# netsys-lab/scion-xdp-br

Measured on AMD Instinct MI355X. Metric: Mpkt/s device-resident hop-field AES-CMAC verify, 64 B SCION packets, higher is better.
Workload: dtype u8; 1 GPU; config 2: 1048576 x 64 B records per GPU per step, single AS key; records_per_gpu=1048576, record_bytes=64, keysel=zero, resident_batches_per_gpu=8, resident_bytes_per_gpu=536870912, parallelism=batch-sharded x1, no collective

## Files before the change

scion-xdp-br_amd/csrc/hfv_aes_dev.h:

```cpp
#pragma once
#include <hip/hip_runtime.h>

#include "hfv_internal.h"

namespace hfv {
#define T0V(i) kTables.t0[i]
#define T0V8(i) T0V(i), T0V(i + 1), T0V(i + 2), T0V(i + 3), T0V(i + 4), T0V(i + 5), T0V(i + 6), T0V(i + 7)
#define T0V64(i) T0V8(i), T0V8(i + 8), T0V8(i + 16), T0V8(i + 24), T0V8(i + 32), T0V8(i + 40), T0V8(i + 48), T0V8(i + 56)
static __constant__ uint32_t c_t0[256] = {T0V64(0), T0V64(64), T0V64(128), T0V64(192)};
#undef T0V64
#undef T0V8
#undef T0V


static __shared__ uint32_t s_tab64[16384];
static __shared__ uint32_t s_tab128[32768];
constexpr uint32_t kTab3Copies = 8;
constexpr uint32_t kTab3Log = kTab3Copies == 32 ? 5 : kTab3Copies == 16 ? 4 : kTab3Copies == 8 ? 3 : kTab3Copies == 4 ? 2 : 99;
static_assert(kTab3Log < 8, "kTab3Copies must be 4, 8, 16 or 32");
static __shared__ uint32_t s_tab32[256 * 2 * kTab3Copies];
static __shared__ uint4 s_keys[kDevKeyRows * HFV_MAX_KEYS];
static __shared__ uint32_t s_valid[8];
static __shared__ uint32_t s_next_tile;

constexpr uint32_t sel_byte(int k) { return 0x0c020400u | (uint32_t(k) << 8); }
constexpr uint32_t SEL_B0 = sel_byte(0), SEL_B1 = sel_byte(1), SEL_B2 = sel_byte(2), SEL_B3 = sel_byte(3);

__device__ __forceinline__ uint32_t rot16(uint32_t x) { return __builtin_amdgcn_alignbit(x, x, 16); }

struct Lane;
template <int TAB, int K>
__device__ __forceinline__ uint32_t tlu(uint32_t w, uint32_t base, const Lane &l);

template <int TAB>
__device__ __forceinline__ void fill_ttab()
{
    if constexpr (TAB == 3) {
#pragma unroll 4
        for (int e = threadIdx.x; e < (int)(256 * 2 * kTab3Copies); e += blockDim.x) {
            uint32_t t = c_t0[(e >> kTab3Log) & 255];
            s_tab32[e] = (e >> (kTab3Log + 8)) ? __builtin_amdgcn_alignbit(t, t, 24) : t;
        }
        return;
    }
    constexpr int kDwords = TAB == 4 ? 32768 : 16384;
    uint32_t *dst = TAB == 4 ? s_tab128 : s_tab64;
#pragma unroll 4
    for (int e = threadIdx.x; e < kDwords; e += blockDim.x) {
        uint32_t t = c_t0[(e >> 6) & 255];
        int rot = 8 * (((e >> 5) & 1) | ((e >> 13) & 2));
        dst[e] = rot ? __builtin_amdgcn_alignbit(t, t, 32 - rot) : t;
    }
}

template <int TAB, class P>
__device__ __forceinline__ void fill_ttab_karg(P t0, uint32_t wave, uint32_t nw)
{
    constexpr uint32_t kChunks = (TAB == 4 ? 131072 : 65536) / 1024;
    constexpr int kMax = (int)((kChunks + 14) / 15);
    const uint32_t lane = threadIdx.x & 63;
    char *lds = TAB == 4 ? reinterpret_cast<char *>(s_tab128) : reinterpret_cast<char *>(s_tab64);
    uint32_t v[kMax];
#pragma unroll
    for (int k = 0; k < kMax; ++k) {
        const uint32_t c = wave + k * nw;
        const uint32_t e = (c << 3) + (lane >> 3);
        v[k] = c < kChunks ? t0[(e >> 1) & 255u] : 0u;
    }
#pragma unroll
    for (int k = 0; k < kMax; ++k) {
        const uint32_t c = wave + k * nw;
        if (c < kChunks) {
            const uint32_t e = (c << 3) + (lane >> 3);
            const uint32_t t = (e & 1u) | (((e >> 9) & 1u) << 1);
            const uint32_t x = t ? __builtin_amdgcn_alignbit(v[k], v[k], 32 - 8 * t) : v[k];
            *reinterpret_cast<uint4 *>(lds + c * 1024 + lane * 16) = make_uint4(x, x, x, x);
        }
    }
}

__device__ __forceinline__ void fill_keys(const DevKeyTable *tab, uint32_t nthr = 0)
{
    const uint32_t n = nthr ? nthr : blockDim.x;
    const uint4 *src = reinterpret_cast<const uint4 *>(tab->rows);
    for (uint32_t e = threadIdx.x; e < kDevKeyRows * HFV_MAX_KEYS; e += n) s_keys[e] = src[e];
    if (threadIdx.x < 8) s_valid[threadIdx.x] = tab->valid[threadIdx.x];
}

struct Lane {
    uint32_t b0, b1, b2, b3;
    uint32_t s0, s1, s2, s3;
    uint32_t f01, f23;
};

template <int TAB, int K>
__device__ __forceinline__ uint32_t tlu(uint32_t w, uint32_t base, const Lane &l)
{
    static_assert(K >= 0 && K < 4, "state byte");
    if constexpr (TAB == 3) {
        const uint32_t a3 = (__builtin_amdgcn_ubfe(w, 8 * K, 8) << (kTab3Log + 2)) | base;
        return *reinterpret_cast<const uint32_t *>(reinterpret_cast<const char *>(s_tab32) + a3);
    }
    const uint32_t a = __builtin_amdgcn_perm(w, base, K == 0 ? l.s0 : K == 1 ? l.s1 : K == 2 ? l.s2 : l.s3);
    const char *t = TAB == 4 ? reinterpret_cast<const char *>(s_tab128) : reinterpret_cast<const char *>(s_tab64);
    return *reinterpret_cast<const uint32_t *>(t + a);
}

__device__ __forceinline__ uint32_t vconst(uint32_t c)
{
    uint32_t r;
    asm("v_mov_b32 %0, %1" : "=v"(r) : "i"(c));
    return r;
}

__device__ __forceinline__ uint32_t xor3(uint32_t a, uint32_t b, uint32_t c)
{
    return __builtin_amdgcn_bitop3_b32(a, b, c, 0x96);
}

template <int TAB, bool PIN = false>
__device__ __forceinline__ void round_full(uint32_t s[4], const uint4 &rk, const Lane &l)
{
    const uint32_t r[4] = {rk.x, rk.y, rk.z, rk.w};
    uint32_t n[4];
#pragma unroll
    for (int c = 0; c < 4; ++c) {
        uint32_t a = tlu<TAB, 0>(s[c], l.b0, l);
        uint32_t b = tlu<TAB, 1>(s[(c + 1) & 3], l.b1, l);
        if constexpr (TAB == 4) {
            uint32_t x = tlu<TAB, 2>(s[(c + 2) & 3], l.b2, l);
            uint32_t d = tlu<TAB, 3>(s[(c + 3) & 3], l.b3, l);
            n[c] = xor3(xor3(a, b, x), d, r[c]);
        } else {
            uint32_t x = tlu<TAB, 2>(s[(c + 2) & 3], l.b0, l);
            uint32_t d = tlu<TAB, 3>(s[(c + 3) & 3], l.b1, l);
            n[c] = xor3(a, b, rot16(xor3(x, d, r[c])));
        }
    }
#pragma unroll
    for (int c = 0; c < 4; ++c) s[c] = n[c];
    if constexpr (TAB == 4 && PIN) {
        __builtin_amdgcn_sched_group_barrier(0x002, 16, 0);
        __builtin_amdgcn_sched_group_barrier(0x100, 16, 0);
        __builtin_amdgcn_sched_group_barrier(0x002, 8, 0);
    }
}

template <int TAB>
__device__ __forceinline__ void round1_macinput(uint32_t s[4], const uint4 &rk1p, const Lane &l)
{
    uint32_t n0, n1, n2, n3;
    if constexpr (TAB == 4) {
        n0 = xor3(tlu<TAB, 1>(s[1], l.b1, l), tlu<TAB, 2>(s[2], l.b2, l), rk1p.x);
        n1 = xor3(xor3(tlu<TAB, 0>(s[1], l.b0, l), tlu<TAB, 1>(s[2], l.b1, l), tlu<TAB, 3>(s[0], l.b3, l)), rk1p.y, 0u);
        n2 = xor3(xor3(tlu<TAB, 1>(s[3], l.b1, l), tlu<TAB, 2>(s[0], l.b2, l), tlu<TAB, 3>(s[1], l.b3, l)), rk1p.z, 0u);
        n3 = xor3(xor3(tlu<TAB, 0>(s[3], l.b0, l), tlu<TAB, 2>(s[1], l.b2, l), tlu<TAB, 3>(s[2], l.b3, l)), rk1p.w, 0u);
    } else {
        n0 = xor3(tlu<TAB, 1>(s[1], l.b1, l), rot16(tlu<TAB, 2>(s[2], l.b0, l)), rk1p.x);
        n1 = xor3(tlu<TAB, 0>(s[1], l.b0, l), tlu<TAB, 1>(s[2], l.b1, l), rk1p.y) ^ rot16(tlu<TAB, 3>(s[0], l.b1, l));
        n2 = xor3(tlu<TAB, 1>(s[3], l.b1, l), rot16(tlu<TAB, 2>(s[0], l.b0, l) ^ tlu<TAB, 3>(s[1], l.b1, l)), rk1p.z);
        n3 = xor3(tlu<TAB, 0>(s[3], l.b0, l), rot16(tlu<TAB, 2>(s[1], l.b0, l) ^ tlu<TAB, 3>(s[2], l.b1, l)), rk1p.w);
    }
// ... 167 lines not shown
```

scion-xdp-br_amd/csrc/hfv_api.cpp:

```cpp
#include <stdarg.h>
#include <stdio.h>
#include <stdlib.h>

#include "hfv_ctx.h"

namespace hfv {

static thread_local char g_err[256];

int fail(int code, const char *fmt, ...)
{
    va_list ap;
    va_start(ap, fmt);
    vsnprintf(g_err, sizeof g_err, fmt, ap);
    va_end(ap);
    return code;
}

}

#ifdef HFV_TEST_HOOKS
static unsigned g_br_grid = 0;
extern "C" int hfv_debug_br_grid(unsigned blocks)
{
// ... 204 lines not shown
    return hfv_key_add(ctx, index, &k);
}

int hfv_key_remove(hfv_ctx *ctx, uint32_t index)
{
    if (!ctx) return fail(-EINVAL, "ctx is NULL");
    if (index >= HFV_MAX_KEYS) return fail(-EINVAL, "key index %u >= %d", index, HFV_MAX_KEYS);
    if (!((ctx->valid[index >> 5] >> (index & 31)) & 1u)) return fail(-ENOENT, "key slot %u is empty", index);
    if (ctx->keymap) {
        int rc = hfv_keymap_erase(ctx->keymap_path, index);
        if (rc) return rc;
    }
    ctx->valid[index >> 5] &= ~(1u << (index & 31));
    memset(&ctx->shadow[index], 0, sizeof(hop_key));
    ctx->dirty = true;
    return 0;
}

int hfv_ctx_attach_keymap(hfv_ctx *ctx, const char *path)
{
    if (!ctx || !path) return fail(-EINVAL, "null argument");
    if (strlen(path) >= sizeof ctx->keymap_path) return fail(-ENAMETOOLONG, "path too long");
    const void *m = nullptr;
    int rc = keymap_open_ro(path, &m);
    if (rc == -ENOENT) {
        rc = keymap_create(path, HFV_KEYMAP_SLOTS);
        if (!rc) rc = keymap_open_ro(path, &m);
    }
    if (rc) return fail(rc, "cannot attach key map %s", path);
    keymap_close(ctx->keymap);
    ctx->keymap = m;
    strcpy(ctx->keymap_path, path);
    ctx->keymap_seq = keymap_snapshot(m, ctx->shadow, ctx->valid);
    ctx->dirty = true;
    return 0;
}

int hfv_key_get(hfv_ctx *ctx, uint32_t index, struct hop_key *out)
{
    if (!ctx || !out) return fail(-EINVAL, "null argument");
    if (index >= HFV_MAX_KEYS) return fail(-EINVAL, "key index %u >= %d", index, HFV_MAX_KEYS);
    if (!((ctx->valid[index >> 5] >> (index & 31)) & 1u)) return fail(-ENOENT, "key slot %u is empty", index);
    *out = ctx->shadow[index];
    return 0;
}

int hfv_key_add_batch(hfv_ctx *ctx, uint32_t first, const struct aes_key *keys, size_t n)
{
    if (!ctx || (!keys && n)) return fail(-EINVAL, "null argument");
    if ((size_t)first + n > HFV_MAX_KEYS) return fail(-EINVAL, "slots %u..%zu exceed %d", first, first + n, HFV_MAX_KEYS);
    if (n == 0) return 0;
    DeviceGuard g(ctx->device);
    SVC_QUIESCE(ctx);
    uint8_t *d_raw = nullptr;
    hop_key *d_hk = nullptr;
    HIP_TRY(hipMalloc((void **)&d_raw, 16 * n));
    if (hipMalloc((void **)&d_hk, sizeof(hop_key) * n) != hipSuccess) {
        (void)hipFree(d_raw);
        return fail(-ENOMEM, "hipMalloc");
    }
    int rc = 0;
    if (hipMemcpyAsync(d_raw, keys, 16 * n, hipMemcpyHostToDevice, ctx->stream) != hipSuccess) rc = -EIO;
    if (!rc && launch_expand_keys(d_raw, n, d_hk, nullptr, 0, ctx->stream) != 0) rc = -EIO;
    hop_key *tmp = (hop_key *)malloc(sizeof(hop_key) * n);
    if (!tmp) rc = -ENOMEM;
    if (!rc && hipMemcpyAsync(tmp, d_hk, sizeof(hop_key) * n, hipMemcpyDeviceToHost, ctx->stream) != hipSuccess) rc = -EIO;
    if (!rc && hipStreamSynchronize(ctx->stream) != hipSuccess) rc = -EIO;
    if (rc) rc = fail(rc, "device key expansion failed");
    for (size_t i = 0; !rc && i < n; ++i) rc = hfv_key_set_hop_key(ctx, first + (uint32_t)i, &tmp[i]);
    free(tmp);
    (void)hipFree(d_raw);
    (void)hipFree(d_hk);
    return rc;
}


static int verify_records(hfv_ctx *ctx, const void *recs, size_t stride, size_t n, uint64_t *pass_bits, void *stream,
                          hipEvent_t ev0, hipEvent_t ev1)
{
    int rc = check_records(ctx, recs, stride, pass_bits);
    if (rc) return rc;
    DeviceGuard g(ctx->device);
    SVC_QUIESCE(ctx);
    return with_tables(ctx, (hipStream_t)stream, "verify_records launch", [&](DevState *ds) {
        return launch_verify_records(batch_geom(ctx), &ds->keys, &ctx->host_img->keys, ctx->keysel, (const uint8_t *)recs,
                                     stride, n, ctx->inf_off, ctx->hf_off, pass_bits, stream, ev0, ev1);
    });
}

int hfv_verify_records(hfv_ctx *ctx, const void *recs, size_t stride, size_t n, uint64_t *pass_bits, void *stream)
{
    if (!ctx) return fail(-EINVAL, "ctx is NULL");
    if (n == 0) return 0;
    return verify_records(ctx, recs, stride, n, pass_bits, stream, nullptr, nullptr);
}

int hfv_verify_records_timed(hfv_ctx *ctx, const void *recs, size_t stride, size_t n, uint64_t *pass_bits,
                             void *stream, float *kernel_ms)
{
    if (!ctx || !kernel_ms) return fail(-EINVAL, "null argument");
    *kernel_ms = 0.0f;
    if (n == 0) return 0;
    return timed(ctx, kernel_ms, [&](hipEvent_t ev0, hipEvent_t ev1) {
        return verify_records(ctx, recs, stride, n, pass_bits, stream, ev0, ev1);
    });
}

static int batches_check(const hfv_ctx *ctx, const struct hfv_batch *b, size_t count)
{
    if (!b && count) return fail(-EINVAL, "null batch list");
    for (size_t i = 0; i < count; ++i) {
        if (b[i].n == 0) continue;
        int rc = check_records(ctx, b[i].recs, b[i].stride, b[i].pass_bits);
        if (rc) return fail_batch(rc, i);
        if (b[i].stride > (1u << 24)) return fail(-EINVAL, "batch %zu: stride %zu > 16 MiB", i, b[i].stride);
        if (b[i].n > ((size_t)1 << 36)) return fail(-EINVAL, "batch %zu: %zu records (at most 2^36)", i, b[i].n);
    }
    return 0;
}

static int batches_launch(hfv_ctx *ctx, const struct hfv_batch *b, size_t count, hipStream_t st, hipEvent_t ev0,
                          hipEvent_t ev1)
{
    size_t last = count;
    while (last > 0 && b[last - 1].n == 0) --last;
    if (ev0) HIP_TRY(hipMemsetAsync(ctx->bat_clk + 4 + kBatchStampBlocks, 0, kBatchStampBlocks * sizeof(uint64_t), st));
    return with_tables(ctx, st, "verify_batches launch", [&](DevState *ds) {
        if (last == 0) return (int)hipSuccess;
        BatchArgs a;
        memset(&a, 0, sizeof a);
        a.tab = &ds->keys;
        a.inf_off = ctx->inf_off;
        a.hf_off = ctx->hf_off;
        a.clk = ctx->bat_clk;
        a.pro = key_prologue(&ctx->host_img->keys);
        for (size_t i = 0;;) {
            a.nb = 0;
            uint64_t tiles = 0;
            for (; i < last && a.nb < kBatchMax; ++i) {
                if (b[i].n == 0) continue;
                const uint64_t t = (b[i].n + 63) / 64;
                if (a.nb && tiles + t > (1ull << 31)) break;
                a.d[a.nb] = {(uint64_t)(uintptr_t)b[i].recs, (uint64_t)(uintptr_t)b[i].pass_bits, (uint64_t)b[i].n,
                             (uint64_t)b[i].stride};
                a.cum[a.nb] = (uint32_t)tiles;
                tiles += t;
                ++a.nb;
            }
            a.cum[a.nb] = (uint32_t)tiles;
            a.total = (uint32_t)tiles;
            const bool fin = i >= last;
            int e = launch_verify_batches(batch_geom(ctx), ctx->keysel, a, st, ev0, fin ? ev1 : nullptr);
            if (e != hipSuccess || fin) return e;
            note_reader(ctx, st);
            ev0 = nullptr;
        }
    });
}

int hfv_verify_batches(hfv_ctx *ctx, const struct hfv_batch *batches, size_t count, void *stream)
{
    if (!ctx) return fail(-EINVAL, "ctx is NULL");
    int rc = batches_check(ctx, batches, count);
    if (rc) return rc;
    DeviceGuard g(ctx->device);
    SVC_QUIESCE(ctx);
    return batches_launch(ctx, batches, count, (hipStream_t)stream, nullptr, nullptr);
}

int hfv_verify_batches_timed(hfv_ctx *ctx, const struct hfv_batch *batches, size_t count, void *stream,
                             float *kernel_ms)
{
    if (!ctx || !kernel_ms) return fail(-EINVAL, "null argument");
    *kernel_ms = 0.0f;
    int rc = batches_check(ctx, batches, count);
    if (rc) return rc;
    size_t nonempty = 0;
    for (size_t i = 0; i < count; ++i) nonempty += batches[i].n != 0;
    if (!nonempty) return 0;
    return timed(ctx, kernel_ms, [&](hipEvent_t ev0, hipEvent_t ev1) {
        SVC_QUIESCE(ctx);
        return batches_launch(ctx, batches, count, (hipStream_t)stream, ev0, ev1);
    });
}


static int frames_check(const hfv_ctx *ctx, const uint8_t *frames, size_t slot, const uint16_t *len, size_t n,
                        const void *recs, size_t stride, const uint8_t *status)
{
    if (!frames || !len || !status) return fail(-EINVAL, "null buffer");
    if ((slot & 7) || slot < 64) return fail(-EINVAL, "slot %zu: must be a multiple of 8, at least 64", slot);
    if (slot > (1u << 24)) return fail(-EINVAL, "slot %zu > 16 MiB", slot);
    int rc = check_records(ctx, recs, stride, recs);
    if (rc) return rc;
    if (stride > (1u << 24)) return fail(-EINVAL, "stride %zu > 16 MiB", stride);
    if (n > ((size_t)1 << 36)) return fail(-EINVAL, "%zu frames (at most 2^36)", n);
    return 0;
}

int hfv_ctx_set_internal_ifindices(hfv_ctx *ctx, const uint32_t *ifindex, size_t n)
{
    if (!ctx) return fail(-EINVAL, "ctx is NULL");
    if (n > kRxSetMax) return fail(-EINVAL, "%zu internal ifindices (at most %u)", n, kRxSetMax);
    if (!ifindex && n) return fail(-EINVAL, "null ifindex list");
    ctx->rx_set.n = (uint32_t)n;
    for (size_t i = 0; i < kRxSetMax; ++i) ctx->rx_set.v[i] = i < n ? ifindex[i] : 0u;
    return 0;
}

static int extract_records_rx(hfv_ctx *ctx, const uint8_t *frames, size_t slot, const uint16_t *len,
                              const uint32_t *ingress_ifindex, size_t n, void *recs, size_t stride, uint8_t *status,
                              void *stream, hipEvent_t ev0, hipEvent_t ev1)
{
    int rc = frames_check(ctx, frames, slot, len, n, recs, stride, status);
    if (rc) return rc;
    DeviceGuard g(ctx->device);
    SVC_QUIESCE(ctx);
    int e = launch_extract_records_rx(frames, slot, len, ingress_ifindex, ctx->rx_set, n, (uint8_t *)recs, stride,
                                      ctx->inf_off, ctx->hf_off, status, stream, ev0, ev1);
    return e == hipSuccess ? 0 : hip_fail((hipError_t)e, "extract_records launch");
}

int hfv_extract_records_rx(hfv_ctx *ctx, const uint8_t *frames, size_t slot, const uint16_t *len,
                           const uint32_t *ingress_ifindex, size_t n, void *recs, size_t stride, uint8_t *status,
                           void *stream)
{
    if (!ctx) return fail(-EINVAL, "ctx is NULL");
    if (n == 0) return 0;
    return extract_records_rx(ctx, frames, slot, len, ingress_ifindex, n, recs, stride, status, stream, nullptr, nullptr);
}

int hfv_extract_records_rx_timed(hfv_ctx *ctx, const uint8_t *frames, size_t slot, const uint16_t *len,
                                 const uint32_t *ingress_ifindex, size_t n, void *recs, size_t stride,
                                 uint8_t *status, void *stream, float *kernel_ms)
{
    if (!ctx || !kernel_ms) return fail(-EINVAL, "null argument");
    *kernel_ms = 0.0f;
// ... 332 lines not shown
```

scion-xdp-br_amd/csrc/hfv_ctx.h:

```cpp
#pragma once
#include <errno.h>
#include <sched.h>
#include <stdio.h>
#include <string.h>

#include <vector>

#include <hip/hip_runtime.h>

#include "hfv_internal.h"

namespace hfv {

static inline int hip_fail(hipError_t e, const char *what)
{
    return fail(-EIO, "%s: %s", what, hipGetErrorString(e));
}

#define HIP_TRY(expr)                                          \
    do {                                                       \
        hipError_t e_ = (expr);                                \
        if (e_ != hipSuccess) return hip_fail(e_, #expr);      \
    } while (0)

// ... 24 lines not shown
    hop_key shadow[HFV_MAX_KEYS];
    uint32_t valid[8] = {0};
    bool dirty = true;
    DevState *host_img = nullptr;
    hipEvent_t img_free = nullptr;
    bool pub_pending = false;
    DevState *dev_tab[2] = {nullptr, nullptr};
    hipStream_t readers[2][8] = {};
    hipEvent_t reader_ev[2][8] = {};
    int nreaders[2] = {0, 0};
    bool readers_overflow[2] = {false, false};
    int active = 0;
    hipStream_t hstream[2] = {nullptr, nullptr};
    uint8_t *h_pin[2] = {nullptr, nullptr};
    uint8_t *d_rec[2] = {nullptr, nullptr};
    uint64_t *h_bits[2] = {nullptr, nullptr};
    uint64_t *d_bits[2] = {nullptr, nullptr};
    size_t host_chunk = 0;
    const void *keymap = nullptr;
    uint32_t keymap_seq = 0xffffffffu;
    char keymap_path[4096] = {0};
    const void *brmap = nullptr;
    uint32_t brmap_seq = 0xffffffffu;
    RxSet rx_set{};
    hipEvent_t tev[2] = {nullptr, nullptr};
    uint64_t *bat_clk = nullptr;
    DevBrConfig br{};
    hfv_br_config cfg_src{};
    size_t brh_win_cap = 0;
    uint8_t *brh_dwin[2] = {nullptr, nullptr};
    uint8_t *brh_dio[2] = {nullptr, nullptr};
    uint8_t *brh_hio[2] = {nullptr, nullptr};
    uint8_t *brh_hwin[2] = {nullptr, nullptr};
    uint64_t *brh_dstats = nullptr;
    struct HostRange {
        uint8_t *host;
        size_t bytes;
        uint8_t *dev;
    };
    HostRange hreg[16] = {};
    int nhreg = 0;
    uint8_t *zc_meta = nullptr;
    size_t zc_cap = 0;
    bool svc_running = false;
    int svc_keysel = HFV_KEYSEL_ZERO;
    uint32_t svc_inf_off = 0, svc_hf_off = 0, svc_idle_ms = 0;
    hipStream_t svc_stream = nullptr;
    SvcShared *svc_host = nullptr;
    SvcShared *svc_host_dev = nullptr;
    SvcDev *svc_dev = nullptr;
    uint32_t svc_launches = 0;
    unsigned svc_grid = 0;
    uint64_t svc_next = 1;
    uint64_t svc_base = 1;
    uint64_t svc_ticket = 1;
    std::vector<uint64_t> svc_lost;
    uint64_t svc_tag = 0;
    bool svc_stop_posted = false;
    bool svc_timing = true;
    bool svc_timed = false;
    hipEvent_t svc_ev[2] = {nullptr, nullptr};
    SvcWeights svc_w = {{kSvcWeightUnit, kSvcWeightUnit, kSvcWeightUnit, kSvcWeightUnit, kSvcWeightUnit,
                         kSvcWeightUnit, kSvcWeightUnit, kSvcWeightUnit},
                        kSvcWeightUnit, {0, 0, 0}};
    SvcWeights svc_w_used = svc_w;
    bool svc_adapt = false;
    std::vector<uint64_t> svc_run_ns;
    uint64_t svc_call_ns[6] = {0, 0, 0, 0, 0, 0};
};

#pragma GCC visibility push(hidden)

int device_numa(int device, cpu_set_t *cpus);
void note_numa(int device);
uint8_t *host_dev_ptr(hfv_ctx *ctx, const void *p, size_t bytes);

int svc_quiesce(hfv_ctx *ctx);
#define SVC_QUIESCE(ctx)                         \
    do {                                         \
        int q_ = svc_quiesce(ctx);               \
        if (q_) return q_;                       \
    } while (0)

int publish_keys(hfv_ctx *ctx, hipStream_t st, DevState **out);
void note_reader(hfv_ctx *ctx, hipStream_t st);
bool own_stream(const hfv_ctx *ctx, hipStream_t st);
int after_launch(hfv_ctx *ctx, hipStream_t st, int err, const char *what);

int check_records(const hfv_ctx *ctx, const void *recs, size_t stride, const void *bits);
#ifdef HFV_TEST_HOOKS
LaunchGeom br_geom(const hfv_ctx *ctx);
LaunchGeom batch_geom(const hfv_ctx *ctx);
#else
#define br_geom(ctx) ((ctx)->geom)
#define batch_geom(ctx) ((ctx)->geom)
#endif

#pragma GCC visibility pop

static inline int fail_batch(int rc, size_t i)
{
    char why[256];
    snprintf(why, sizeof why, "%s", hfv_last_error());
    return fail(rc, "batch %zu: %s", i, why);
}

template <class Launch>
static inline int with_tables(hfv_ctx *ctx, hipStream_t st, const char *what, Launch launch)
{
    DevState *ds;
    int rc = publish_keys(ctx, st, &ds);
    if (rc) return rc;
    return after_launch(ctx, st, launch(ds), what);
}
```

scion-xdp-br_amd/csrc/hfv_host_path.cpp:

```cpp
#include <pthread.h>
#include <stdlib.h>

#include <condition_variable>
#include <functional>
#include <mutex>
#include <thread>

#include "hfv_ctx.h"

static constexpr size_t kHostRec = 24;

static int host_threads()
{
    static const int t = [] {
        const char *e = getenv("HFV_HOST_THREADS");
        int v = e ? atoi(e) : 0;
        if (v <= 0) {
            unsigned hc = std::thread::hardware_concurrency();
            v = hc ? (int)(hc < 8 ? hc : 8) : 4;
        }
        return v;
    }();
    return t;
}
// ... 338 lines not shown
    for (size_t i = 0; i < n; ++i) nretry += action[i] == HFV_BR_ACTION_RETRY;
    if (nretry) {
        rc = brh_buffers(ctx, slot);
        if (rc) return rc;
        uint8_t *bounce = nullptr;
        size_t cap = nretry < kBrChunk ? nretry : kBrChunk;
        HIP_TRY(hipHostMalloc((void **)&bounce, cap * slot + cap * 8, hipHostMallocDefault));
        uint16_t *blen = (uint16_t *)(bounce + cap * slot);
        uint32_t *bif = (uint32_t *)(bounce + cap * slot + cap * 2);
        size_t *idx = (size_t *)malloc(cap * sizeof(size_t));
        size_t i = 0;
        while (rc == 0 && i < n) {
            size_t cnt = 0;
            for (; i < n && cnt < cap; ++i) {
                if (action[i] != HFV_BR_ACTION_RETRY) continue;
                memcpy(bounce + cnt * slot, frames + i * slot, slot);
                blen[cnt] = len[i];
                bif[cnt] = ingress_ifindex[i];
                idx[cnt++] = i;
            }
            if (!cnt) break;
            rc = brh_chunk(ctx, 0, bounce, slot, slot, slot, blen, bif, cnt);
            if (rc == 0 && hipStreamSynchronize(ctx->hstream[0]) != hipSuccess) rc = fail(-EIO, "retry chunk");
            for (size_t k = 0; rc == 0 && k < cnt; ++k) {
                size_t j = idx[k];
                memcpy(frames + j * slot, ctx->brh_hwin[0] + k * slot, slot);
                action[j] = ctx->brh_hio[0][kBrChunk * 6 + k];
                verdict[j] = ctx->brh_hio[0][kBrChunk * 7 + k];
                memcpy(&egress_ifindex[j], ctx->brh_hio[0] + kBrChunk * 8 + 4 * k, 4);
            }
        }
        free(idx);
        (void)hipHostFree(bounce);
        if (rc) return rc;
    }
    return brh_add_stats(ctx, stats);
}

int hfv_host_register(hfv_ctx *ctx, void *ptr, size_t bytes)
{
    if (!ctx || !ptr || !bytes) return fail(-EINVAL, "bad argument");
    if (ctx->nhreg == 16) return fail(-ENOMEM, "at most 16 registered host buffers per ctx");
    DeviceGuard g(ctx->device);
    HIP_TRY(hipHostRegister(ptr, bytes, hipHostRegisterMapped));
    void *dev = nullptr;
    hipError_t e = hipHostGetDevicePointer(&dev, ptr, 0);
    if (e != hipSuccess) {
        (void)hipHostUnregister(ptr);
        return hip_fail(e, "hipHostGetDevicePointer");
    }
    ctx->hreg[ctx->nhreg++] = {(uint8_t *)ptr, bytes, (uint8_t *)dev};
    return 0;
}

int hfv_host_unregister(hfv_ctx *ctx, void *ptr)
{
    if (!ctx || !ptr) return fail(-EINVAL, "bad argument");
    DeviceGuard g(ctx->device);
    for (int i = 0; i < ctx->nhreg; ++i) {
        if (ctx->hreg[i].host != ptr) continue;
        HIP_TRY(hipDeviceSynchronize());
        HIP_TRY(hipHostUnregister(ptr));
        ctx->hreg[i] = ctx->hreg[--ctx->nhreg];
        return 0;
    }
    return fail(-EINVAL, "buffer was not registered with this ctx");
}

static int verify_records_zero_copy(hfv_ctx *ctx, const uint8_t *drecs, size_t stride, size_t n, uint64_t *pass_bits)
{
    hipStream_t st = ctx->stream;
    const size_t words = (n + 63) / 64;
    uint64_t *dbits = (uint64_t *)host_dev_ptr(ctx, pass_bits, words * 8);
    if (!dbits) {
        if (ctx->zc_cap < words * 8) {
            if (ctx->zc_meta) (void)hipFree(ctx->zc_meta);
            ctx->zc_meta = nullptr;
            ctx->zc_cap = 0;
            HIP_TRY(hipMalloc((void **)&ctx->zc_meta, words * 8));
            ctx->zc_cap = words * 8;
        }
        dbits = (uint64_t *)ctx->zc_meta;
    }
    int rc = with_tables(ctx, st, "verify_records launch (zero-copy)", [&](DevState *ds) {
        return launch_verify_records(batch_geom(ctx), &ds->keys, &ctx->host_img->keys, ctx->keysel, drecs, stride, n,
                                     ctx->inf_off, ctx->hf_off, dbits, st, nullptr, nullptr, true);
    });
    if (rc) return rc;
    if (dbits == (uint64_t *)ctx->zc_meta) HIP_TRY(hipMemcpyAsync(pass_bits, dbits, words * 8, hipMemcpyDeviceToHost, st));
    HIP_TRY(hipStreamSynchronize(st));
    return 0;
}

int hfv_verify_records_host(hfv_ctx *ctx, const void *recs, size_t stride, size_t n, uint64_t *pass_bits)
{
    if (!ctx) return fail(-EINVAL, "ctx is NULL");
    if (n == 0) return 0;
    int rc = check_records(ctx, recs, stride, pass_bits);
    if (rc) return rc;
    DeviceGuard g(ctx->device);
    SVC_QUIESCE(ctx);
    if (const uint8_t *drecs = host_dev_ptr(ctx, recs, (n - 1) * stride + ctx->hf_off + 12))
        return verify_records_zero_copy(ctx, drecs, stride, n, pass_bits);
    const size_t chunk = (size_t)1 << 18;
    if (ctx->host_chunk < chunk * kHostRec) {
        for (int i = 0; i < 2; ++i) {
            if (ctx->h_pin[i]) (void)hipHostFree(ctx->h_pin[i]);
            if (ctx->d_rec[i]) (void)hipFree(ctx->d_rec[i]);
            if (ctx->h_bits[i]) (void)hipHostFree(ctx->h_bits[i]);
            if (ctx->d_bits[i]) (void)hipFree(ctx->d_bits[i]);
            ctx->h_pin[i] = ctx->d_rec[i] = nullptr;
            ctx->h_bits[i] = ctx->d_bits[i] = nullptr;
            if (!ctx->hstream[i]) HIP_TRY(hipStreamCreateWithFlags(&ctx->hstream[i], hipStreamNonBlocking));
            HIP_TRY(hipHostMalloc((void **)&ctx->h_pin[i], chunk * kHostRec, hipHostMallocDefault));
            HIP_TRY(hipMalloc((void **)&ctx->d_rec[i], chunk * kHostRec));
            HIP_TRY(hipHostMalloc((void **)&ctx->h_bits[i], chunk / 8, hipHostMallocDefault));
            HIP_TRY(hipMalloc((void **)&ctx->d_bits[i], chunk / 8));
        }
        ctx->host_chunk = chunk * kHostRec;
    }
    size_t nchunks = (n + chunk - 1) / chunk;
    size_t pending_words[2] = {0, 0};
    size_t pending_first[2] = {0, 0};
    for (size_t c = 0; c < nchunks + 2; ++c) {
        int slot = (int)(c & 1);
        hipStream_t st = ctx->hstream[slot];
        if (c >= 2) {
            HIP_TRY(hipStreamSynchronize(st));
            memcpy(pass_bits + pending_first[slot], ctx->h_bits[slot], pending_words[slot] * 8);
        }
        if (c >= nchunks) continue;
        size_t first = c * chunk, cnt = n - first < chunk ? n - first : chunk;
        gather_hf(ctx->h_pin[slot], (const uint8_t *)recs + first * stride, stride, ctx->inf_off, ctx->hf_off, cnt);
        HIP_TRY(hipMemcpyAsync(ctx->d_rec[slot], ctx->h_pin[slot], cnt * kHostRec, hipMemcpyHostToDevice, st));
        rc = with_tables(ctx, st, "verify_records launch", [&](DevState *ds) {
            return launch_verify_records(batch_geom(ctx), &ds->keys, &ctx->host_img->keys, ctx->keysel, ctx->d_rec[slot],
                                         kHostRec, cnt, 0, 8, ctx->d_bits[slot], st);
        });
        if (rc) return rc;
        size_t words = (cnt + 63) / 64;
        HIP_TRY(hipMemcpyAsync(ctx->h_bits[slot], ctx->d_bits[slot], words * 8, hipMemcpyDeviceToHost, st));
        pending_words[slot] = words;
        pending_first[slot] = first / 64;
    }
    return 0;
}

}
```

scion-xdp-br_amd/csrc/hfv_publish.cpp:

```cpp
#include <utility>

#include "hfv_ctx.h"

#ifndef HFV_PUB_FENCE
#define HFV_PUB_FENCE 1
#endif
#ifndef HFV_READER_FENCE
#define HFV_READER_FENCE 1
#endif

#ifdef HFV_TEST_HOOKS
static uint32_t g_pub_delay_us = 0;
extern "C" int hfv_debug_publish_delay(uint32_t us)
{
    g_pub_delay_us = us;
    return 0;
}
#else
static constexpr uint32_t g_pub_delay_us = 0;
#endif

int publish_keys(hfv_ctx *ctx, hipStream_t st, DevState **out)
{
    if (ctx->keymap) {
        uint32_t seq = keymap_seq(ctx->keymap);
        if (seq != ctx->keymap_seq) {
            ctx->keymap_seq = keymap_snapshot(ctx->keymap, ctx->shadow, ctx->valid);
            ctx->dirty = true;
        }
    }
    if (ctx->brmap) {
        uint32_t seq = brcfg_seq(ctx->brmap);
        if (seq != ctx->brmap_seq) {
            hfv_br_config cfg;
            uint32_t detached = 0, feat_off = 0;
            ctx->brmap_seq = brcfg_snapshot(ctx->brmap, &cfg, &detached, &feat_off);
            if (br_config_check(&cfg) != 0)
                return fail(-EINVAL, "attached router config holds counts past the fixed capacity; "
                                     "previous tables kept");
            const uint32_t off = ctx->br.hf_check_off;
            ctx->cfg_src = cfg;
            compile_br_config(&cfg, &ctx->br);
            ctx->br.hf_check_off = off;
            ctx->br.detached = detached;
            ctx->br.feat_off = feat_off & (HFV_BR_NO_IPV4 | HFV_BR_NO_IPV6 | HFV_BR_NO_SCION_PATH);
            ctx->dirty = true;
        }
    }
    if (ctx->dirty) {
        int next = ctx->active ^ 1;
        HIP_TRY(hipEventSynchronize(ctx->img_free));
        for (uint32_t k = 0; k < HFV_MAX_KEYS; ++k) {
            uint32_t dk[4 * kDevKeyRows], t[8];
            if ((ctx->valid[k >> 5] >> (k & 31)) & 1u) {
                compile_dev_key(&ctx->shadow[k], dk);
                compile_dev_sched(&ctx->shadow[k], t);
            } else {
                memset(dk, 0, sizeof dk);
                memset(t, 0, sizeof t);
            }
            for (int r = 0; r < kDevKeyRows; ++r) memcpy(ctx->host_img->keys.rows[r][k], dk + 4 * r, 16);
            memcpy(ctx->host_img->keys.sched[0][k], t, 16);
            memcpy(ctx->host_img->keys.sched[1][k], t + 4, 16);
        }
        memcpy(ctx->host_img->keys.valid, ctx->valid, sizeof ctx->valid);
        ctx->host_img->br = ctx->br;
        if (!HFV_READER_FENCE) {
        } else if (ctx->readers_overflow[next]) {
            HIP_TRY(hipDeviceSynchronize());
        } else {
            for (int r = 0; r < ctx->nreaders[next]; ++r) {
                hipStream_t rs = ctx->readers[next][r];
                if (rs == st) continue;
                if (own_stream(ctx, rs)) HIP_TRY(hipEventRecord(ctx->reader_ev[next][r], rs));
                HIP_TRY(hipStreamWaitEvent(st, ctx->reader_ev[next][r], 0));
            }
        }
        ctx->nreaders[next] = 0;
        ctx->readers_overflow[next] = false;
        if (g_pub_delay_us) HIP_TRY((hipError_t)launch_debug_spin(st, g_pub_delay_us));
        HIP_TRY(hipMemcpyAsync(ctx->dev_tab[next], ctx->host_img, sizeof(DevState), hipMemcpyHostToDevice, st));
        HIP_TRY(hipEventRecord(ctx->img_free, st));
        ctx->active = next;
        ctx->dirty = false;
        ctx->pub_pending = true;
    } else if (HFV_PUB_FENCE && ctx->pub_pending) {
        if (hipEventQuery(ctx->img_free) == hipSuccess) ctx->pub_pending = false;
        else HIP_TRY(hipStreamWaitEvent(st, ctx->img_free, 0));
    }
    *out = ctx->dev_tab[ctx->active];
    return 0;
}

bool own_stream(const hfv_ctx *ctx, hipStream_t st)
{
    return st && (st == ctx->stream || st == ctx->svc_stream || st == ctx->hstream[0] || st == ctx->hstream[1]);
}

void note_reader(hfv_ctx *ctx, hipStream_t st)
{
    const int a = ctx->active;
    int r = 0;
    while (r < ctx->nreaders[a] && ctx->readers[a][r] != st) ++r;
    if (r == ctx->nreaders[a]) {
        if (r == 8) {
            ctx->readers_overflow[a] = true;
            return;
        }
        ctx->readers[a][ctx->nreaders[a]++] = st;
    }
    if (!own_stream(ctx, st) && hipEventRecord(ctx->reader_ev[a][r], st) != hipSuccess) ctx->readers_overflow[a] = true;
}

int after_launch(hfv_ctx *ctx, hipStream_t st, int err, const char *what)
{
    if (err != hipSuccess) return hip_fail((hipError_t)err, what);
    note_reader(ctx, st);
    return 0;
}

void hfv::forget_stream(hfv_ctx *ctx, void *stream)
{
    for (int a = 0; a < 2; ++a)
        for (int r = 0; r < ctx->nreaders[a];)
            if (ctx->readers[a][r] == (hipStream_t)stream) {
                const int last = --ctx->nreaders[a];
                ctx->readers[a][r] = ctx->readers[a][last];
                std::swap(ctx->reader_ev[a][r], ctx->reader_ev[a][last]);
            } else {
                ++r;
            }
}
```

scion-xdp-br_amd/csrc/hfv_verify_dev.h:

```cpp
#pragma once
#include <hip/hip_runtime.h>

#include "hfv_aes_dev.h"
#include "hfv_internal.h"

namespace hfv {

typedef uint32_t u32x2 __attribute__((ext_vector_type(2)));

typedef __attribute__((address_space(1))) uint8_t GlobalU8;
typedef __attribute__((address_space(1))) uint64_t GlobalU64;

struct RecWords {
    uint2 inf;
    uint2 hfa;
    uint32_t hfb;
};

template <bool NT, class B>
__device__ __forceinline__ RecWords load_tile(const B &b, uint64_t tile, uint32_t lane, uint32_t inf_off,
                                              uint32_t hf_off)
{
    const uint64_t first = tile * 64;
    const uint64_t left = b.n - 1 - first;
    const uint32_t lim = left < 63 ? (uint32_t)left : 63u;
    const uint32_t off = (lane < lim ? lane : lim) * (uint32_t)b.stride;
    const GlobalU8 *p = (const GlobalU8 *)(b.recs + first * b.stride) + off;
    typedef const __attribute__((address_space(1))) u32x2 *P2;
    typedef const __attribute__((address_space(1))) uint32_t *P1;
    auto ld = [](auto q) { return NT ? __builtin_nontemporal_load(q) : *q; };
    RecWords r;
    const u32x2 x = ld(reinterpret_cast<P2>(p + inf_off));
    const u32x2 y = ld(reinterpret_cast<P2>(p + hf_off));
    r.hfb = ld(reinterpret_cast<P1>(p + hf_off + 8));
    r.inf = make_uint2(x.x, x.y);
    r.hfa = make_uint2(y.x, y.y);
    return r;
}

__device__ __forceinline__ void rec_macinput(const RecWords &r, uint32_t w[4])
{
    uint32_t noncons_mask = (r.inf.x & 1u) ? 0u : 0xffff0000u;
    w[0] = (r.inf.x & 0xffff0000u) ^ (r.hfa.y & noncons_mask);
    w[1] = r.inf.y;
    w[2] = r.hfa.x & 0xffffff00u;
    w[3] = r.hfa.y & 0xffffu;
}

__device__ __forceinline__ uint32_t rec_key_slot(const RecWords &r)
{
    return (r.inf.x & 1u) ? (r.hfa.x >> 24) : ((r.hfa.y >> 8) & 0xffu);
}

__device__ __forceinline__ bool rec_tag_matches(const RecWords &r, uint32_t t0, uint32_t t1)
{
    uint32_t e0 = __builtin_amdgcn_alignbit(r.hfb, r.hfa.y, 16);
    uint32_t e1 = r.hfb >> 16;
    return t0 == e0 && ((t1 ^ e1) & 0xffffu) == 0;
}

template <int KEYSEL, bool PIN = false>
__device__ __forceinline__ uint64_t verify_tile(const RecWords &r, bool in, const Lane &l, const UniformKey *ukey)
{
    uint32_t w[4], t0, t1;
    rec_macinput(r, w);
    bool ok = in;
    if constexpr (KEYSEL == HFV_KEYSEL_ZERO) {
        cmac48_macinput<4, UniformKey, PIN>(w, *ukey, l, t0, t1);
    } else {
        const uint32_t slot = rec_key_slot(r);
        cmac48_sched(w, slot, l, t0, t1);
        ok = ok && slot_valid(slot);
    }
    return __ballot(ok && rec_tag_matches(r, t0, t1));
}

template <int KEYSEL, class P>
__device__ __forceinline__ void fill_block(P t0, const DevKeyTable *tab, uint32_t nthr)
{
    if (threadIdx.x < nthr) fill_ttab_karg<4>(t0, threadIdx.x >> 6, nthr >> 6);
    if constexpr (KEYSEL == HFV_KEYSEL_IFID) {
        if (threadIdx.x < nthr) fill_keys5(tab, nthr);
    }
}

constexpr int kBlock = 1024;
constexpr uint32_t kWaves = kBlock / 64;

static inline unsigned grid_for(uint64_t n, int block, int num_cus, int per_cu)
{
    uint64_t tiles = (n + 63) / 64;
    uint64_t blocks = (tiles + block / 64 - 1) / (block / 64);
    uint64_t cap = (uint64_t)num_cus * (uint64_t)(per_cu > 0 ? per_cu : 1);
    if (blocks > cap) blocks = cap;
    return (unsigned)(blocks ? blocks : 1);
}

}
```

scion-xdp-br_amd/csrc/hfv_verify_kernels.hip:

```cpp
#include <hip/hip_runtime.h>
#include <string.h>

#include <hip/hip_ext.h>

#include "hfv_verify_dev.h"

namespace hfv {

__device__ __forceinline__ RecWords load_rec(const uint8_t *recs, uint64_t stride, uint64_t i, uint64_t last,
                                             uint32_t inf_off, uint32_t hf_off)
{
    RecWords r;
    const GlobalU8 *p = (const GlobalU8 *)(recs) + (i < last ? i : last) * stride;
    typedef const __attribute__((address_space(1))) u32x2 *P2;
    typedef const __attribute__((address_space(1))) uint32_t *P1;
    const u32x2 a = __builtin_nontemporal_load(reinterpret_cast<P2>(p + inf_off));
    const u32x2 b = __builtin_nontemporal_load(reinterpret_cast<P2>(p + hf_off));
    r.hfb = __builtin_nontemporal_load(reinterpret_cast<P1>(p + hf_off + 8));
    r.inf = make_uint2(a.x, a.y);
    r.hfa = make_uint2(b.x, b.y);
    return r;
}

template <int KEYSEL, int DYN, int STAMP = 0>
// ... 21 lines not shown
    fill_block<KEYSEL>(ka.t0, tab, kBlock);
    __syncthreads();
    const Lane l = lane_bases();
    if constexpr (STAMP) {
        if (lane == 0) {
            st[1] = __builtin_amdgcn_s_memrealtime();
            st[12] = __builtin_amdgcn_s_memtime();
        }
    }
    if constexpr (KEYSEL == HFV_KEYSEL_ZERO) {
        if (!ukey.ok) {
            for (uint64_t tt = t; tt < count; tt += stride_t)
                if (lane == 0) bits[b0 + tt] = 0;
            return;
        }
    }
    uint64_t st_word = 0, st_tile = 0;
    uint32_t stashed = 0;
    int nst = 0;
    while (t < count) {
        uint64_t nt;
        if constexpr (DYN) {
            uint32_t c = 0;
            if (lane == 0) c = atomicAdd(&s_next_tile, 1u);
            nt = wave_uniform(c);
        } else {
            nt = t + stride_t;
        }
        RecWords nxt = load_rec(recs, stride, (b0 + nt) * 64 + lane, last, inf_off, hf_off);
        const uint64_t ballot = verify_tile<KEYSEL, true>(cur, (b0 + t) * 64 + lane < n, l, &ukey);
        if (lane == stashed) {
            st_word = ballot;
            st_tile = b0 + t;
        }
        if (++stashed == 64) {
            ((GlobalU64 *)bits)[st_tile] = st_word;
            stashed = 0;
        }
        if constexpr (STAMP) {
            if (lane == 0 && nst < 10) st[2 + nst] = __builtin_amdgcn_s_memrealtime();
            ++nst;
        }
        cur = nxt;
        t = nt;
    }
    if (lane < stashed) ((GlobalU64 *)bits)[st_tile] = st_word;
    if constexpr (STAMP) {
        if (lane == 0) {
            st[13] = __builtin_amdgcn_s_memtime();
            st[15] = __builtin_amdgcn_s_memrealtime();
            st[14] = (uint64_t)__builtin_amdgcn_s_getreg((31 << 11) | 4) |
                     ((uint64_t)__builtin_amdgcn_s_getreg((15 << 11) | 20) << 32);
        }
    }
}

typedef const __attribute__((address_space(4))) BatchArgs *BArgs;

struct BatchTile {
    uint64_t recs, bits, n, stride;
    uint32_t lo, hi;
    uint32_t j;
};

__device__ __forceinline__ void batch_enter(BArgs a, uint32_t j, BatchTile &b)
{
    b.j = j;
    b.recs = a->d[j].recs;
    b.bits = a->d[j].bits;
    b.n = a->d[j].n;
    b.stride = a->d[j].stride;
    b.lo = a->cum[j];
    b.hi = a->cum[j + 1];
}

__device__ __forceinline__ void batch_map(BArgs a, uint32_t g, BatchTile &b)
{
    if (g < b.hi) return;
    uint32_t j = b.j + 1;
    while (g >= a->cum[j + 1]) ++j;
    batch_enter(a, j, b);
}

__device__ __forceinline__ RecWords batch_load(const BatchTile &b, uint32_t g, uint32_t lane, uint32_t inf_off,
                                               uint32_t hf_off)
{
    return load_tile<true>(b, g - b.lo, lane, inf_off, hf_off);
}

#ifndef HFV_MUT_TILEDEAL
#define HFV_MUT_TILEDEAL 0
#endif
template <int KEYSEL>
__global__ __launch_bounds__(kBlock) void k_verify_batches(const BatchArgs args)
{
    const BArgs a = (BArgs)__builtin_amdgcn_kernarg_segment_ptr();
    (void)args;
    const uint32_t lane = threadIdx.x & 63;
    const uint32_t wv = wave_uniform(threadIdx.x / 64);
    const uint32_t total = a->total;
    const uint32_t b0 = (uint32_t)((uint64_t)total * blockIdx.x / gridDim.x);
    const uint32_t b1 = (uint32_t)((uint64_t)total * (blockIdx.x + 1) / gridDim.x);
    if (b1 == b0) return;
    const uint32_t last = b1 - 1;
    const uint32_t inf_off = a->inf_off, hf_off = a->hf_off;
    UniformKey ukey(a->pro.key0, a->pro.key0_ok);
    if (threadIdx.x == 0 && a->clk) {
        a->clk[4 + blockIdx.x] = __builtin_amdgcn_s_memrealtime();
        if (blockIdx.x == 0) {
            a->clk[0] = __builtin_amdgcn_s_memtime();
            a->clk[1] = __builtin_amdgcn_s_memrealtime();
        }
    }
#if HFV_MUT_TILEDEAL == 4
    if (threadIdx.x == 0) s_next_tile = kWaves + 1;
#else
    if (threadIdx.x == 0) s_next_tile = kWaves;
#endif
    auto at = [&](uint32_t x) { return x < b1 ? x : last; };
    auto claim = [&]() -> uint32_t {
        uint32_t c = 0;
        if (lane == 0) c = atomicAdd(&s_next_tile, 1u);
        return b0 + wave_uniform(c);
    };
    constexpr int S = 2;
    RecWords buf[S];
    BatchTile bt[S];
    uint32_t gg[S];
    gg[0] = b0 + wv;
    bt[0].hi = 0;
    bt[0].j = ~0u;
    batch_map(a, at(gg[0]), bt[0]);
    buf[0] = batch_load(bt[0], at(gg[0]), lane, inf_off, hf_off);
    fill_block<KEYSEL>(a->pro.t0, a->tab, kBlock);
    __syncthreads();
    const Lane l = lane_bases();
    uint64_t st_word = 0, st_addr = 0;
    uint32_t stashed = 0;
    const bool fail_closed = KEYSEL == HFV_KEYSEL_ZERO && !ukey.ok;
    if (gg[0] >= b1 || fail_closed) goto done;
    for (;;) {
#pragma unroll
        for (int u = 0; u < S; ++u) {
            const int in_slot = (u + 1) % S;
            gg[in_slot] = claim();
            bt[in_slot] = bt[u];
            batch_map(a, at(gg[in_slot]), bt[in_slot]);
            buf[in_slot] = batch_load(bt[in_slot], at(gg[in_slot]), lane, inf_off, hf_off);
            const uint64_t rec = (uint64_t)(gg[u] - bt[u].lo) * 64 + lane;
#if HFV_MUT_TILEDEAL == 2
            const uint64_t n_own = bt[in_slot].n;
#else
            const uint64_t n_own = bt[u].n;
#endif
            const uint64_t ballot = verify_tile<KEYSEL, true>(buf[u], rec < n_own, l, &ukey);
            if (lane == stashed) {
                st_word = ballot;
                st_addr = bt[u].bits + (uint64_t)(gg[u] - bt[u].lo) * 8;
            }
            if (++stashed == 64) {
#if HFV_MUT_TILEDEAL == 1
                if (lane != 63)
#endif
                *(GlobalU64 *)st_addr = st_word;
                stashed = 0;
            }
            if (gg[(u + 1) % S] >= b1) goto done;
        }
    }
done:
    if (lane < stashed) *(GlobalU64 *)st_addr = st_word;
    if (fail_closed) {
        for (uint32_t g = b0 + wv; g < b1; g += kWaves) {
            batch_map(a, g, bt[0]);
            if (lane == 0) *(GlobalU64 *)(bt[0].bits + (uint64_t)(g - bt[0].lo) * 8) = 0;
#if HFV_MUT_TILEDEAL == 3
            break;
#endif
        }
    }
    if (lane == 0 && a->clk)
        __hip_atomic_fetch_max(&a->clk[4 + kBatchStampBlocks + blockIdx.x], __builtin_amdgcn_s_memrealtime(),
                               __ATOMIC_RELAXED, __HIP_MEMORY_SCOPE_AGENT);
    if (blockIdx.x == 0 && threadIdx.x == 0 && a->clk) {
        a->clk[2] = __builtin_amdgcn_s_memtime();
        a->clk[3] = __builtin_amdgcn_s_memrealtime();
    }
}

int launch_verify_batches(const LaunchGeom &g, int keysel, const BatchArgs &args, void *stream, void *ev_start,
                          void *ev_stop)
{
    auto k = keysel == HFV_KEYSEL_IFID ? k_verify_batches<HFV_KEYSEL_IFID> : k_verify_batches<HFV_KEYSEL_ZERO>;
    uint64_t blocks = args.total;
    if (blocks > (uint64_t)g.num_cus) blocks = (uint64_t)g.num_cus;
    if (g.batch_grid_cap && g.batch_grid_cap < blocks) blocks = g.batch_grid_cap;
    hipExtLaunchKernelGGL(k, dim3((unsigned)(blocks ? blocks : 1)), dim3(kBlock), 0, (hipStream_t)stream,
                          (hipEvent_t)ev_start, (hipEvent_t)ev_stop, 0u, args);
    return (int)hipGetLastError();
}

KeyPrologue key_prologue(const DevKeyTable *host_keys)
{
    KeyPrologue ka;
    memset(&ka, 0, sizeof ka);
    if (host_keys) {
        for (int r = 0; r < kDevKeyRows; ++r) memcpy(&ka.key0[4 * r], host_keys->rows[r][0], 16);
        ka.key0_ok = host_keys->valid[0] & 1u;
    }
    memcpy(ka.t0, kTables.t0, sizeof ka.t0);
    return ka;
}

int launch_verify_records(const LaunchGeom &g, const DevKeyTable *tab, const DevKeyTable *host_keys, int keysel,
                          const uint8_t *recs,
                          size_t stride, size_t n, uint32_t inf_off, uint32_t hf_off, uint64_t *bits, void *stream,
                          void *ev_start, void *ev_stop, bool interleaved)
// ... 39 lines not shown
```

Before: 95800 Mpkt/s.

## Split table fill into load/store, binary-search first batch, skip reader fences for zero keysel

Splits the LDS T-table fill into a kernarg load phase issued before the first record load and a store phase after it, so the table reads overlap the first tile's global load. The first tile's batch index is now found with a binary search over the cumulative tile offsets instead of a linear walk. On the host side, launches with the zero key selector no longer record reader events or wait on the publish fence, which cuts per-launch host and stream-dependency overhead. This relies on the zero-keysel kernels never reading the device key table; holding the table values in registers longer may add register pressure.

```diff
diff --git a/scion-xdp-br_amd/csrc/hfv_aes_dev.h b/scion-xdp-br_amd/csrc/hfv_aes_dev.h
--- a/scion-xdp-br_amd/csrc/hfv_aes_dev.h
+++ b/scion-xdp-br_amd/csrc/hfv_aes_dev.h
@@ -78,6 +78,46 @@
         }
     }
 }
+
+template <int TAB>
+struct TtabFill {
+    static constexpr uint32_t kChunks = (TAB == 4 ? 131072 : 65536) / 1024;
+    static constexpr int kMax = (int)((kChunks + 14) / 15);
+    uint32_t v[kMax];
+};
+
+template <int TAB, class P>
+__device__ __forceinline__ void ttab_karg_load(P t0, uint32_t wave, uint32_t nw, TtabFill<TAB> &f)
+{
+    constexpr uint32_t kChunks = TtabFill<TAB>::kChunks;
+    const uint32_t lane = threadIdx.x & 63;
+#pragma unroll
+    for (int k = 0; k < TtabFill<TAB>::kMax; ++k) {
+        const uint32_t c = wave + k * nw;
+        const uint32_t e = (c << 3) + (lane >> 3);
+        f.v[k] = c < kChunks ? t0[(e >> 1) & 255u] : 0u;
+    }
+}
+
+template <int TAB>
+__device__ __forceinline__ void ttab_karg_store(uint32_t wave, uint32_t nw, const TtabFill<TAB> &f)
+{
+    constexpr uint32_t kChunks = TtabFill<TAB>::kChunks;
+    const uint32_t lane = threadIdx.x & 63;
+    char *lds = TAB == 4 ? reinterpret_cast<char *>(s_tab128) : reinterpret_cast<char *>(s_tab64);
+    const uint32_t *v = f.v;
+#pragma unroll
+    for (int k = 0; k < TtabFill<TAB>::kMax; ++k) {
+        const uint32_t c = wave + k * nw;
+        if (c < kChunks) {
+            const uint32_t e = (c << 3) + (lane >> 3);
+            const uint32_t t = (e & 1u) | (((e >> 9) & 1u) << 1);
+            const uint32_t x = t ? __builtin_amdgcn_alignbit(v[k], v[k], 32 - 8 * t) : v[k];
+            *reinterpret_cast<uint4 *>(lds + c * 1024 + lane * 16) = make_uint4(x, x, x, x);
+        }
+    }
+}
+
 
 __device__ __forceinline__ void fill_keys(const DevKeyTable *tab, uint32_t nthr = 0)
 {
diff --git a/scion-xdp-br_amd/csrc/hfv_api.cpp b/scion-xdp-br_amd/csrc/hfv_api.cpp
--- a/scion-xdp-br_amd/csrc/hfv_api.cpp
+++ b/scion-xdp-br_amd/csrc/hfv_api.cpp
@@ -310,7 +310,8 @@
     if (rc) return rc;
     DeviceGuard g(ctx->device);
     SVC_QUIESCE(ctx);
-    return with_tables(ctx, (hipStream_t)stream, "verify_records launch", [&](DevState *ds) {
+    const bool reader = launch_reads_tables(ctx->keysel);
+    return with_tables(ctx, (hipStream_t)stream, "verify_records launch", reader, [&](DevState *ds) {
         return launch_verify_records(batch_geom(ctx), &ds->keys, &ctx->host_img->keys, ctx->keysel, (const uint8_t *)recs,
                                      stride, n, ctx->inf_off, ctx->hf_off, pass_bits, stream, ev0, ev1);
     });
@@ -353,7 +354,8 @@
     size_t last = count;
     while (last > 0 && b[last - 1].n == 0) --last;
     if (ev0) HIP_TRY(hipMemsetAsync(ctx->bat_clk + 4 + kBatchStampBlocks, 0, kBatchStampBlocks * sizeof(uint64_t), st));
-    return with_tables(ctx, st, "verify_batches launch", [&](DevState *ds) {
+    const bool reader = launch_reads_tables(ctx->keysel);
+    return with_tables(ctx, st, "verify_batches launch", reader, [&](DevState *ds) {
         if (last == 0) return (int)hipSuccess;
         BatchArgs a;
         memset(&a, 0, sizeof a);
@@ -380,7 +382,7 @@
             const bool fin = i >= last;
             int e = launch_verify_batches(batch_geom(ctx), ctx->keysel, a, st, ev0, fin ? ev1 : nullptr);
             if (e != hipSuccess || fin) return e;
-            note_reader(ctx, st);
+            if (reader) note_reader(ctx, st);
             ev0 = nullptr;
         }
     });
diff --git a/scion-xdp-br_amd/csrc/hfv_ctx.h b/scion-xdp-br_amd/csrc/hfv_ctx.h
--- a/scion-xdp-br_amd/csrc/hfv_ctx.h
+++ b/scion-xdp-br_amd/csrc/hfv_ctx.h
@@ -130,10 +130,10 @@
         if (q_) return q_;                       \
     } while (0)
 
-int publish_keys(hfv_ctx *ctx, hipStream_t st, DevState **out);
+int publish_keys(hfv_ctx *ctx, hipStream_t st, DevState **out, bool reader = true);
 void note_reader(hfv_ctx *ctx, hipStream_t st);
 bool own_stream(const hfv_ctx *ctx, hipStream_t st);
-int after_launch(hfv_ctx *ctx, hipStream_t st, int err, const char *what);
+int after_launch(hfv_ctx *ctx, hipStream_t st, int err, const char *what, bool reader = true);
 
 int check_records(const hfv_ctx *ctx, const void *recs, size_t stride, const void *bits);
 #ifdef HFV_TEST_HOOKS
@@ -153,11 +153,19 @@
     return fail(rc, "batch %zu: %s", i, why);
 }
 
+static inline bool launch_reads_tables(int keysel) { return keysel != HFV_KEYSEL_ZERO; }
+
+template <class Launch>
+static inline int with_tables(hfv_ctx *ctx, hipStream_t st, const char *what, bool reader, Launch launch)
+{
+    DevState *ds;
+    int rc = publish_keys(ctx, st, &ds, reader);
+    if (rc) return rc;
+    return after_launch(ctx, st, launch(ds), what, reader);
+}
+
 template <class Launch>
 static inline int with_tables(hfv_ctx *ctx, hipStream_t st, const char *what, Launch launch)
 {
-    DevState *ds;
-    int rc = publish_keys(ctx, st, &ds);
-    if (rc) return rc;
-    return after_launch(ctx, st, launch(ds), what);
+    return with_tables(ctx, st, what, true, launch);
 }
diff --git a/scion-xdp-br_amd/csrc/hfv_host_path.cpp b/scion-xdp-br_amd/csrc/hfv_host_path.cpp
--- a/scion-xdp-br_amd/csrc/hfv_host_path.cpp
+++ b/scion-xdp-br_amd/csrc/hfv_host_path.cpp
@@ -444,7 +444,8 @@
         }
         dbits = (uint64_t *)ctx->zc_meta;
     }
-    int rc = with_tables(ctx, st, "verify_records launch (zero-copy)", [&](DevState *ds) {
+    const bool reader = launch_reads_tables(ctx->keysel);
+    int rc = with_tables(ctx, st, "verify_records launch (zero-copy)", reader, [&](DevState *ds) {
         return launch_verify_records(batch_geom(ctx), &ds->keys, &ctx->host_img->keys, ctx->keysel, drecs, stride, n,
                                      ctx->inf_off, ctx->hf_off, dbits, st, nullptr, nullptr, true);
     });
@@ -495,7 +496,7 @@
         size_t first = c * chunk, cnt = n - first < chunk ? n - first : chunk;
         gather_hf(ctx->h_pin[slot], (const uint8_t *)recs + first * stride, stride, ctx->inf_off, ctx->hf_off, cnt);
         HIP_TRY(hipMemcpyAsync(ctx->d_rec[slot], ctx->h_pin[slot], cnt * kHostRec, hipMemcpyHostToDevice, st));
-        rc = with_tables(ctx, st, "verify_records launch", [&](DevState *ds) {
+        rc = with_tables(ctx, st, "verify_records launch", launch_reads_tables(ctx->keysel), [&](DevState *ds) {
             return launch_verify_records(batch_geom(ctx), &ds->keys, &ctx->host_img->keys, ctx->keysel, ctx->d_rec[slot],
                                          kHostRec, cnt, 0, 8, ctx->d_bits[slot], st);
         });
diff --git a/scion-xdp-br_amd/csrc/hfv_publish.cpp b/scion-xdp-br_amd/csrc/hfv_publish.cpp
--- a/scion-xdp-br_amd/csrc/hfv_publish.cpp
+++ b/scion-xdp-br_amd/csrc/hfv_publish.cpp
@@ -20,7 +20,7 @@
 static constexpr uint32_t g_pub_delay_us = 0;
 #endif
 
-int publish_keys(hfv_ctx *ctx, hipStream_t st, DevState **out)
+int publish_keys(hfv_ctx *ctx, hipStream_t st, DevState **out, bool reader)
 {
     if (ctx->keymap) {
         uint32_t seq = keymap_seq(ctx->keymap);
@@ -84,7 +84,7 @@
         ctx->active = next;
         ctx->dirty = false;
         ctx->pub_pending = true;
-    } else if (HFV_PUB_FENCE && ctx->pub_pending) {
+    } else if (HFV_PUB_FENCE && ctx->pub_pending && reader) {
         if (hipEventQuery(ctx->img_free) == hipSuccess) ctx->pub_pending = false;
         else HIP_TRY(hipStreamWaitEvent(st, ctx->img_free, 0));
     }
@@ -112,10 +112,10 @@
     if (!own_stream(ctx, st) && hipEventRecord(ctx->reader_ev[a][r], st) != hipSuccess) ctx->readers_overflow[a] = true;
 }
 
-int after_launch(hfv_ctx *ctx, hipStream_t st, int err, const char *what)
+int after_launch(hfv_ctx *ctx, hipStream_t st, int err, const char *what, bool reader)
 {
     if (err != hipSuccess) return hip_fail((hipError_t)err, what);
-    note_reader(ctx, st);
+    if (reader) note_reader(ctx, st);
     return 0;
 }
 
diff --git a/scion-xdp-br_amd/csrc/hfv_verify_dev.h b/scion-xdp-br_amd/csrc/hfv_verify_dev.h
--- a/scion-xdp-br_amd/csrc/hfv_verify_dev.h
+++ b/scion-xdp-br_amd/csrc/hfv_verify_dev.h
@@ -87,6 +87,13 @@
 constexpr int kBlock = 1024;
 constexpr uint32_t kWaves = kBlock / 64;
 
+template <int KEYSEL>
+__device__ __forceinline__ void fill_block_store(const TtabFill<4> &f, const DevKeyTable *tab)
+{
+    ttab_karg_store<4>(threadIdx.x >> 6, kWaves, f);
+    if constexpr (KEYSEL == HFV_KEYSEL_IFID) fill_keys5(tab, kBlock);
+}
+
 static inline unsigned grid_for(uint64_t n, int block, int num_cus, int per_cu)
 {
     uint64_t tiles = (n + 63) / 64;
diff --git a/scion-xdp-br_amd/csrc/hfv_verify_kernels.hip b/scion-xdp-br_amd/csrc/hfv_verify_kernels.hip
--- a/scion-xdp-br_amd/csrc/hfv_verify_kernels.hip
+++ b/scion-xdp-br_amd/csrc/hfv_verify_kernels.hip
@@ -127,6 +127,21 @@
     batch_enter(a, j, b);
 }
 
+__device__ __forceinline__ uint32_t batch_find(BArgs a, uint32_t nb, uint32_t g)
+{
+    uint32_t lo = 0, len = nb;
+    while (len > 1) {
+        const uint32_t half = len >> 1;
+        if (g >= a->cum[lo + half]) {
+            lo += half;
+            len -= half;
+        } else {
+            len = half;
+        }
+    }
+    return lo;
+}
+
 __device__ __forceinline__ RecWords batch_load(const BatchTile &b, uint32_t g, uint32_t lane, uint32_t inf_off,
                                                uint32_t hf_off)
 {
@@ -143,13 +158,12 @@
     (void)args;
     const uint32_t lane = threadIdx.x & 63;
     const uint32_t wv = wave_uniform(threadIdx.x / 64);
-    const uint32_t total = a->total;
+    const uint32_t total = a->total, nb = a->nb;
     const uint32_t b0 = (uint32_t)((uint64_t)total * blockIdx.x / gridDim.x);
     const uint32_t b1 = (uint32_t)((uint64_t)total * (blockIdx.x + 1) / gridDim.x);
     if (b1 == b0) return;
     const uint32_t last = b1 - 1;
     const uint32_t inf_off = a->inf_off, hf_off = a->hf_off;
-    UniformKey ukey(a->pro.key0, a->pro.key0_ok);
     if (threadIdx.x == 0 && a->clk) {
         a->clk[4 + blockIdx.x] = __builtin_amdgcn_s_memrealtime();
         if (blockIdx.x == 0) {
@@ -172,12 +186,13 @@
     RecWords buf[S];
     BatchTile bt[S];
     uint32_t gg[S];
+    TtabFill<4> t0w;
+    ttab_karg_load<4>(a->pro.t0, threadIdx.x >> 6, kWaves, t0w);
     gg[0] = b0 + wv;
-    bt[0].hi = 0;
-    bt[0].j = ~0u;
-    batch_map(a, at(gg[0]), bt[0]);
+    UniformKey ukey(a->pro.key0, a->pro.key0_ok);
+    batch_enter(a, batch_find(a, nb, at(gg[0])), bt[0]);
     buf[0] = batch_load(bt[0], at(gg[0]), lane, inf_off, hf_off);
-    fill_block<KEYSEL>(a->pro.t0, a->tab, kBlock);
+    fill_block_store<KEYSEL>(t0w, a->tab);
     __syncthreads();
     const Lane l = lane_bases();
     uint64_t st_word = 0, st_addr = 0;
```

Measured after the change: 98990 Mpkt/s, median of 6. 1.03x the previous value.
